# Arthur151/ROMP

Measured on NVIDIA H100. Metric: frames/sec 512x512 ROMP-HRNet32 (whole hot path), higher is better.
Workload: dtype bf16

## Files before the change

romp_b200/csrc/conv_bottleneck_tc.cu:

```cuda
#include "conv_tc.cuh"
#include "tc_device.cuh"

namespace b200romp {

namespace {

constexpr int kBnThreads = 384;
constexpr int kRowB = 128;
constexpr int kHaloW = 10, kHaloH = 18;
constexpr int kChunks = 4;
constexpr int kRing = 2;
constexpr int kW1Bytes = kChunks * 64 * kRowB;
constexpr int kW2Bytes = 9 * 64 * kRowB;
constexpr int kW3Bytes = 256 * kRowB;
constexpr int kStagePayload = kHaloH * kHaloW * kRowB;
constexpr int kStageBytes = 192 * kRowB;
constexpr int kMidBytes = 192 * kRowB;
constexpr int kT2Bytes = 128 * kRowB;
constexpr int kSmemBytes = kW1Bytes + kW2Bytes + kW3Bytes + kRing * kStageBytes + kMidBytes + kT2Bytes + 1024  +
                           1024 ;
static_assert(kSmemBytes <= 227 * 1024, "fused bottleneck does not fit shared memory");

__device__ __forceinline__ void consumers_bar_sync() { asm volatile("bar.sync 1, 256;" ::: "memory"); }

__device__ __forceinline__ void st_shared_b32(uint32_t addr, uint32_t v) {
  asm volatile("st.shared.b32 [%0], %1;" ::"r"(addr), "r"(v) : "memory");
}
template <typename T>
__device__ __forceinline__ T opaque(T v) {
  uint64_t u = (uint64_t)v;
  asm volatile("mov.b64 %0, %0;" : "+l"(u));
  return (T)u;
}
__device__ __forceinline__ uint32_t pack_bf16x2(float a, float b) {
  const __nv_bfloat162 v = __floats2bfloat162_rn(a, b);
  return *reinterpret_cast<const uint32_t*>(&v);
}

}

template <bool STORE_MIDS>
__global__ void __launch_bounds__(kBnThreads, 1)
conv_bottleneck_tc_kernel(const __grid_constant__ CUtensorMap tmap, const ConvParams p, const uint8_t* __restrict__ w1pack,
                          const uint8_t* __restrict__ w2pack, const uint8_t* __restrict__ w3pack, const float* __restrict__ bias1,
                          const float* __restrict__ bias2, BottleneckMids mids, int tiles_x, int tiles_y, int num_tiles) {
  extern __shared__ uint8_t smem_raw[];
  uint8_t* smem = reinterpret_cast<uint8_t*>((reinterpret_cast<uintptr_t>(smem_raw) + 1023) & ~(uintptr_t)1023);
  uint8_t* sW1 = smem;
  uint8_t* sW2 = sW1 + kW1Bytes;
  uint8_t* sW3 = sW2 + kW2Bytes;
  uint8_t* sA = sW3 + kW3Bytes;
  uint8_t* sMid = sA + kRing * kStageBytes;
  uint8_t* sT2 = sMid + kMidBytes;
  uint64_t* full = reinterpret_cast<uint64_t*>(sT2 + kT2Bytes);
  uint64_t* empty = full + kRing;
  uint64_t* w_full = empty + kRing;

  const int warp = threadIdx.x >> 5;
  if (threadIdx.x == 0) {
    for (int i = 0; i < kRing; ++i) {
      mbar_init(&full[i], 1);
      mbar_init(&empty[i], 8);
    }
    mbar_init(w_full, 1);
    fence_barrier_init();
  }
  __syncthreads();
  pdl_trigger();
  const int per_frame = tiles_x * tiles_y;

  if (warp == 0) {
    if (elect_one()) {
      mbar_arrive_expect_tx(w_full, kW1Bytes + kW2Bytes + kW3Bytes);
      bulk_copy_g2s(sW1, w1pack, kW1Bytes, w_full);
      for (int t = 0; t < 9; ++t) bulk_copy_g2s(sW2 + t * 64 * kRowB, w2pack + (size_t)t * 64 * kRowB, 64 * kRowB, w_full);
      bulk_copy_g2s(sW3, w3pack, kW3Bytes, w_full);
      pdl_wait();
      const uint64_t pol = l2_policy_stream();
      int stage = 0;
      uint32_t phase = 0;
      for (int tile = blockIdx.x; tile < num_tiles; tile += gridDim.x) {
        const int n = tile / per_frame, rem = tile % per_frame;
        const int y0 = (rem / tiles_x) * 16, x0 = (rem % tiles_x) * 8;
        for (int c = 0; c < kChunks; ++c) {
          mbar_wait(&empty[stage], phase ^ 1);
          mbar_arrive_expect_tx(&full[stage], kStagePayload);
          tma_load_4d(sA + stage * kStageBytes, &tmap, &full[stage], c * 64, x0 - 1, y0 - 1, n, pol);
          if (++stage == kRing) { stage = 0; phase ^= 1; }
        }
      }
    }
  } else if (warp >= 4) {
    const int g = (warp >> 2) - 1, t = threadIdx.x & 127, w = t >> 5, l = t & 31;
    pdl_wait();
    mbar_wait(w_full, 0);
    const int cl = 2 * (l & 3);
    int stage = 0;
    uint32_t phase = 0;
    for (int tile = blockIdx.x; tile < num_tiles; tile += gridDim.x) {
      const uint32_t w1_base = opaque(smem_u32(sW1)), w2_base = opaque(smem_u32(sW2)), w3_base = opaque(smem_u32(sW3)),
                     a_base = opaque(smem_u32(sA)), mid_base = opaque(smem_u32(sMid)), t2_base = opaque(smem_u32(sT2));
      const float* b1p = opaque(bias1);
      const float* b2p = opaque(bias2);
      const float* b3p = opaque(p.bias);
      const int n = tile / per_frame, rem = tile % per_frame;
      const int y0 = (rem / tiles_x) * 16, x0 = (rem % tiles_x) * 8;

      float acc[32], acc_b[16];
#pragma unroll
      for (int j = 0; j < 32; ++j) acc[j] = 0.f;
#pragma unroll
      for (int j = 0; j < 16; ++j) acc_b[j] = 0.f;
      uint32_t scale_d = 0;
      int prev = -1;
#pragma unroll
      for (int c = 0; c < kChunks; ++c) {
        mbar_wait(&full[stage], phase);
        const uint32_t a_st = a_base + (uint32_t)(stage * kStageBytes);
        const uint32_t b_ch = w1_base + (uint32_t)(c * 64 * kRowB);
        wgmma_fence();
#pragma unroll
        for (int k = 0; k < 4; ++k) {
          wgmma_n64(acc, make_smem_desc(a_st + 64 * g * kRowB + k * 32, 8 * kRowB, kSw128),
                    make_smem_desc(b_ch + k * 32, 8 * kRowB, kSw128), scale_d, false);
          wgmma_n32(acc_b, make_smem_desc(a_st + 128 * kRowB + k * 32, 8 * kRowB, kSw128),
                    make_smem_desc(b_ch + 32 * g * kRowB + k * 32, 8 * kRowB, kSw128), scale_d, false);
          scale_d = 1;
        }
        wgmma_commit();
        if (prev >= 0) {
          wgmma_wait<1>();
          if (l == 0) mbar_arrive(&empty[prev]);
        }
        prev = stage;
        if (++stage == kRing) { stage = 0; phase ^= 1; }
      }
      wgmma_wait<0>();
      if (l == 0) mbar_arrive(&empty[prev]);

      consumers_bar_sync();
      auto mid_store = [&](int m, int j, float a, float b) {
        const int my = m / kHaloW, mx = m % kHaloW;
        const bool inside = my < kHaloH && (unsigned)(y0 - 1 + my) < (unsigned)p.Hout && (unsigned)(x0 - 1 + mx) < (unsigned)p.Wout;
        if (!inside) a = b = 0.f;
        const uint32_t v = pack_bf16x2(a, b);
        st_shared_b32(mid_base + m * kRowB + ((j ^ (m & 7)) << 4) + 2 * cl, v);
        if constexpr (STORE_MIDS) {
          if (mids.t1 != nullptr && my >= 1 && my <= 16 && mx >= 1 && mx <= 8) {
            const size_t pix = ((size_t)n * p.Hout + y0 - 1 + my) * p.Wout + x0 - 1 + mx;
            *reinterpret_cast<uint32_t*>(mids.t1 + pix * mids.t1_C + 8 * j + cl) = v;
          }
        }
      };
#pragma unroll
      for (int e = 0; e < 2; ++e) {
        const int m = 64 * g + 16 * w + (l >> 2) + 8 * e;
#pragma unroll
        for (int j = 0; j < 8; ++j) {
          const int c = 8 * j + cl;
          mid_store(m, j, fmaxf(acc[4 * j + 2 * e] + __ldg(b1p + c), 0.f), fmaxf(acc[4 * j + 2 * e + 1] + __ldg(b1p + c + 1), 0.f));
        }
        const int mb = 128 + 16 * w + (l >> 2) + 8 * e;
#pragma unroll
        for (int j = 0; j < 4; ++j) {
          const int c = 32 * g + 8 * j + cl;
          mid_store(mb, 4 * g + j, fmaxf(acc_b[4 * j + 2 * e] + __ldg(b1p + c), 0.f),
                    fmaxf(acc_b[4 * j + 2 * e + 1] + __ldg(b1p + c + 1), 0.f));
        }
      }
      fence_proxy_async();
      consumers_bar_sync();

      float acc2[32];
#pragma unroll
      for (int j = 0; j < 32; ++j) acc2[j] = 0.f;
      scale_d = 0;
      wgmma_fence();
#pragma unroll
      for (int tap = 0; tap < 9; ++tap) {
        const uint32_t a_tap = mid_base + (uint32_t)(((8 * g + tap / 3) * kHaloW + tap % 3) * kRowB);
        const uint32_t b_tap = w2_base + (uint32_t)(tap * 64 * kRowB);
#pragma unroll
        for (int k = 0; k < 4; ++k) {
          wgmma_n64(acc2, make_smem_desc(a_tap + k * 32, kHaloW * kRowB, kSw128), make_smem_desc(b_tap + k * 32, 8 * kRowB, kSw128),
                    scale_d, false);
          scale_d = 1;
        }
      }
      wgmma_commit();
      wgmma_wait<0>();

#pragma unroll
      for (int e = 0; e < 2; ++e) {
        const int m = 64 * g + 16 * w + (l >> 2) + 8 * e;
#pragma unroll
        for (int j = 0; j < 8; ++j) {
          const int c = 8 * j + cl;
          const uint32_t v = pack_bf16x2(fmaxf(acc2[4 * j + 2 * e] + __ldg(b2p + c), 0.f), fmaxf(acc2[4 * j + 2 * e + 1] + __ldg(b2p + c + 1), 0.f));
          st_shared_b32(t2_base + m * kRowB + ((j ^ (m & 7)) << 4) + 2 * cl, v);
          if constexpr (STORE_MIDS) {
            if (mids.t2 != nullptr) {
              const size_t pix = ((size_t)n * p.Hout + y0 + 8 * g + 2 * w + e) * p.Wout + x0 + (l >> 2);
              *reinterpret_cast<uint32_t*>(mids.t2 + pix * mids.t2_C + c) = v;
            }
          }
        }
      }
      fence_proxy_async();
      wg_bar_sync(2 + g);

      const __nv_bfloat16* res = reinterpret_cast<const __nv_bfloat16*>(p.res);
      __nv_bfloat16* out = reinterpret_cast<__nv_bfloat16*>(p.out);
#pragma unroll 1
      for (int h = 0; h < 2; ++h) {
        float acc3[64];
#pragma unroll
        for (int j = 0; j < 64; ++j) acc3[j] = 0.f;
        wgmma_fence();
#pragma unroll
        for (int k = 0; k < 4; ++k)
          wgmma_n128_bf16(acc3, make_smem_desc(t2_base + 64 * g * kRowB + k * 32, 8 * kRowB, kSw128),
                          make_smem_desc(w3_base + h * 128 * kRowB + k * 32, 8 * kRowB, kSw128), k > 0 ? 1u : 0u);
        wgmma_commit();
        uint32_t rv[2][16];
#pragma unroll
        for (int e = 0; e < 2; ++e) {
          const size_t pix = ((size_t)n * p.Hout + y0 + 8 * g + 2 * w + e) * p.Wout + x0 + (l >> 2);
          const uint32_t* r = reinterpret_cast<const uint32_t*>(res + pix * p.res_C + p.res_c_off + 128 * h + cl);
#pragma unroll
          for (int j = 0; j < 16; ++j) rv[e][j] = r[4 * j];
        }
        wgmma_wait<0>();
#pragma unroll
        for (int e = 0; e < 2; ++e) {
          const size_t pix = ((size_t)n * p.Hout + y0 + 8 * g + 2 * w + e) * p.Wout + x0 + (l >> 2);
          __nv_bfloat162* o = reinterpret_cast<__nv_bfloat162*>(out + pix * p.out_C + p.out_c_off + 128 * h + cl);
#pragma unroll
          for (int j = 0; j < 16; ++j) {
            const int c = 128 * h + 8 * j + cl;
            float a = acc3[4 * j + 2 * e] + __ldg(b3p + c), b = acc3[4 * j + 2 * e + 1] + __ldg(b3p + c + 1);
            const float2 r = res_pair(rv[e][j]);
            a += r.x; b += r.y;
            o[4 * j] = __floats2bfloat162_rn(fmaxf(a, 0.f), fmaxf(b, 0.f));
          }
        }
      }
    }
  }
}

bool tc_bottleneck_supported(const ConvParams& p) {
  if (p.in_dtype != B200ROMP_BF16 || p.out_dtype != B200ROMP_BF16 || p.res_dtype != B200ROMP_BF16) return false;
  if (p.cin != 256 || p.cout != 256 || p.up != 1 || p.out_nchw || p.pow_channel >= 0 || p.input_norm || !p.relu) return false;
  if (p.Hin != p.Hout || p.Win != p.Wout || p.Hout % 16 != 0 || p.Wout % 8 != 0) return false;
  if (p.in_C % 8 != 0 || p.in_c_off % 8 != 0 || p.out_C % 8 != 0 || p.out_c_off % 8 != 0) return false;
  if (p.res != p.in || p.res_C != p.in_C || p.res_c_off != p.in_c_off || p.res_broadcast) return false;
  return (reinterpret_cast<uintptr_t>(p.in) & 15) == 0;
}

int tc_bottleneck_prepare(const ConvParams& p, const float* w1_oihw, const float* b1, const float* w2_oihw, const float* b2,
                          const float* w3_oihw, int sm_count, TcConvPlan* plan, std::vector<void*>* allocs) {
  plan->kind = 70;
  plan->eb = 2;
  plan->cin = plan->cout = 256;
  plan->nt = 256;
  plan->grid_x = sm_count;
  plan->grid_y = 1;
  plan->stages = kRing;
  plan->smem_bytes = kSmemBytes;
  int rc = tc_pack_weights(w1_oihw, 256, 64, 1, 64, &plan->d_wpack, allocs, kRowB, 2);
  if (!rc) rc = tc_pack_weights(w2_oihw, 64, 64, 9, 64, &plan->d_wpack2, allocs, kRowB, 2);
  if (!rc) rc = tc_pack_weights(w3_oihw, 64, 256, 1, 256, &plan->d_wpack3, allocs, kRowB, 2);
  if (rc) return rc;
  plan->d_bias1 = static_cast<const float*>(upload(b1, 64 * sizeof(float), allocs));
  plan->d_bias2 = static_cast<const float*>(upload(b2, 64 * sizeof(float), allocs));
  if (!plan->d_bias1 || !plan->d_bias2) return B200ROMP_ECUDA;
  rc = tc_encode_nhwc_input(&plan->tmap_in, p, 2, 64, kHaloW, kHaloH, CU_TENSOR_MAP_SWIZZLE_128B, "conv_bottleneck_tc");
  if (rc) return rc;
  B2R_CUDA_OK(cudaFuncSetAttribute(conv_bottleneck_tc_kernel<false>, cudaFuncAttributeMaxDynamicSharedMemorySize, kSmemBytes));
  B2R_CUDA_OK(cudaFuncSetAttribute(conv_bottleneck_tc_kernel<true>, cudaFuncAttributeMaxDynamicSharedMemorySize, kSmemBytes));
  return B200ROMP_OK;
}

int tc_bottleneck_launch(const TcConvPlan& plan, const ConvParams& p, const BottleneckMids& mids, cudaStream_t stream) {
  const int tiles_x = p.Wout / 8, tiles_y = p.Hout / 16;
  const int num_tiles = tiles_x * tiles_y * p.B;
  const dim3 grid(std::min(plan.grid_x, num_tiles));
  auto kern = mids.t1 != nullptr || mids.t2 != nullptr ? conv_bottleneck_tc_kernel<true> : conv_bottleneck_tc_kernel<false>;
  B2R_CUDA_OK(tc_launch(kern, grid, kBnThreads, plan.smem_bytes, stream, plan.tmap_in, p, reinterpret_cast<const uint8_t*>(plan.d_wpack),
                        reinterpret_cast<const uint8_t*>(plan.d_wpack2), reinterpret_cast<const uint8_t*>(plan.d_wpack3),
                        plan.d_bias1, plan.d_bias2, mids, tiles_x, tiles_y, num_tiles));
  return B200ROMP_OK;
}

}
```

Baseline: 3602.

## Overlap next-tile conv1 with conv3 epilogue, rebalance registers, vectorize residual I/O

The fused bottleneck kernel now starts the first two conv1 chunks of the next tile right after conv2, so the TMA ring and the tensor cores stay busy during the conv2/conv3 epilogues. Producer warps give up registers via setmaxnreg and consumers gain them, to fit the larger live state. The residual loads and output stores move from 32-bit scattered accesses to 128-bit vectors, using a quad shuffle transpose, and an alignment check on the output pointer is added. The cost is more register pressure, extra shuffles, and a more complex ring-phase ordering across tiles.

```diff
diff --git a/romp_b200/csrc/conv_bottleneck_tc.cu b/romp_b200/csrc/conv_bottleneck_tc.cu
--- a/romp_b200/csrc/conv_bottleneck_tc.cu
+++ b/romp_b200/csrc/conv_bottleneck_tc.cu
@@ -31,6 +31,19 @@
   uint64_t u = (uint64_t)v;
   asm volatile("mov.b64 %0, %0;" : "+l"(u));
   return (T)u;
+}
+constexpr int kProducerRegs = 40, kConsumerRegs = 232;
+template <int R>
+__device__ __forceinline__ void setmaxnreg_dec() { asm volatile("setmaxnreg.dec.sync.aligned.u32 %0;" ::"n"(R)); }
+template <int R>
+__device__ __forceinline__ void setmaxnreg_inc() { asm volatile("setmaxnreg.inc.sync.aligned.u32 %0;" ::"n"(R)); }
+__device__ __forceinline__ void quad_transpose(uint32_t (&m)[4], int q) {
+  const bool b1 = q & 2, b0 = q & 1;
+  uint32_t s0 = __shfl_xor_sync(0xffffffffu, b1 ? m[0] : m[2], 2), s1 = __shfl_xor_sync(0xffffffffu, b1 ? m[1] : m[3], 2);
+  if (b1) { m[0] = s0; m[1] = s1; } else { m[2] = s0; m[3] = s1; }
+  s0 = __shfl_xor_sync(0xffffffffu, b0 ? m[0] : m[1], 1);
+  s1 = __shfl_xor_sync(0xffffffffu, b0 ? m[2] : m[3], 1);
+  if (b0) { m[0] = s0; m[2] = s1; } else { m[1] = s0; m[3] = s1; }
 }
 __device__ __forceinline__ uint32_t pack_bf16x2(float a, float b) {
   const __nv_bfloat162 v = __floats2bfloat162_rn(a, b);
@@ -69,8 +82,9 @@
   pdl_trigger();
   const int per_frame = tiles_x * tiles_y;
 
-  if (warp == 0) {
-    if (elect_one()) {
+  if (warp < 4) {
+    setmaxnreg_dec<kProducerRegs>();
+    if (warp == 0 && elect_one()) {
       mbar_arrive_expect_tx(w_full, kW1Bytes + kW2Bytes + kW3Bytes);
       bulk_copy_g2s(sW1, w1pack, kW1Bytes, w_full);
       for (int t = 0; t < 9; ++t) bulk_copy_g2s(sW2 + t * 64 * kRowB, w2pack + (size_t)t * 64 * kRowB, 64 * kRowB, w_full);
@@ -90,53 +104,60 @@
         }
       }
     }
-  } else if (warp >= 4) {
+  } else {
+    setmaxnreg_inc<kConsumerRegs>();
     const int g = (warp >> 2) - 1, t = threadIdx.x & 127, w = t >> 5, l = t & 31;
     pdl_wait();
     mbar_wait(w_full, 0);
     const int cl = 2 * (l & 3);
     int stage = 0;
     uint32_t phase = 0;
+    float acc[32], acc_b[16];
+    auto conv1_chunks = [&](int c0, int c1) {
+      const uint32_t w1_base = opaque(smem_u32(sW1)), a_base = opaque(smem_u32(sA));
+      if (c0 == 0) {
+#pragma unroll
+        for (int j = 0; j < 32; ++j) acc[j] = 0.f;
+#pragma unroll
+        for (int j = 0; j < 16; ++j) acc_b[j] = 0.f;
+      }
+      int prev = -1;
+#pragma unroll
+      for (int c = c0; c < c1; ++c) {
+        mbar_wait(&full[stage], phase);
+        const uint32_t a_st = a_base + (uint32_t)(stage * kStageBytes);
+        const uint32_t b_ch = w1_base + (uint32_t)(c * 64 * kRowB);
+        wgmma_fence();
+#pragma unroll
+        for (int k = 0; k < 4; ++k) {
+          const uint32_t scale_d = c > 0 || k > 0 ? 1u : 0u;
+          wgmma_n64(acc, make_smem_desc(a_st + 64 * g * kRowB + k * 32, 8 * kRowB, kSw128),
+                    make_smem_desc(b_ch + k * 32, 8 * kRowB, kSw128), scale_d, false);
+          wgmma_n32(acc_b, make_smem_desc(a_st + 128 * kRowB + k * 32, 8 * kRowB, kSw128),
+                    make_smem_desc(b_ch + 32 * g * kRowB + k * 32, 8 * kRowB, kSw128), scale_d, false);
+        }
+        wgmma_commit();
+        if (prev >= 0) {
+          wgmma_wait<1>();
+          if (l == 0) mbar_arrive(&empty[prev]);
+        }
+        prev = stage;
+        if (++stage == kRing) { stage = 0; phase ^= 1; }
+      }
+      wgmma_wait<0>();
+      if (l == 0) mbar_arrive(&empty[prev]);
+    };
+    if (blockIdx.x < num_tiles) conv1_chunks(0, kRing);
     for (int tile = blockIdx.x; tile < num_tiles; tile += gridDim.x) {
-      const uint32_t w1_base = opaque(smem_u32(sW1)), w2_base = opaque(smem_u32(sW2)), w3_base = opaque(smem_u32(sW3)),
-                     a_base = opaque(smem_u32(sA)), mid_base = opaque(smem_u32(sMid)), t2_base = opaque(smem_u32(sT2));
+      const uint32_t w2_base = opaque(smem_u32(sW2)), w3_base = opaque(smem_u32(sW3)), mid_base = opaque(smem_u32(sMid)),
+                     t2_base = opaque(smem_u32(sT2));
       const float* b1p = opaque(bias1);
       const float* b2p = opaque(bias2);
       const float* b3p = opaque(p.bias);
       const int n = tile / per_frame, rem = tile % per_frame;
       const int y0 = (rem / tiles_x) * 16, x0 = (rem % tiles_x) * 8;
 
-      float acc[32], acc_b[16];
-#pragma unroll
-      for (int j = 0; j < 32; ++j) acc[j] = 0.f;
-#pragma unroll
-      for (int j = 0; j < 16; ++j) acc_b[j] = 0.f;
-      uint32_t scale_d = 0;
-      int prev = -1;
-#pragma unroll
-      for (int c = 0; c < kChunks; ++c) {
-        mbar_wait(&full[stage], phase);
-        const uint32_t a_st = a_base + (uint32_t)(stage * kStageBytes);
-        const uint32_t b_ch = w1_base + (uint32_t)(c * 64 * kRowB);
-        wgmma_fence();
-#pragma unroll
-        for (int k = 0; k < 4; ++k) {
-          wgmma_n64(acc, make_smem_desc(a_st + 64 * g * kRowB + k * 32, 8 * kRowB, kSw128),
-                    make_smem_desc(b_ch + k * 32, 8 * kRowB, kSw128), scale_d, false);
-          wgmma_n32(acc_b, make_smem_desc(a_st + 128 * kRowB + k * 32, 8 * kRowB, kSw128),
-                    make_smem_desc(b_ch + 32 * g * kRowB + k * 32, 8 * kRowB, kSw128), scale_d, false);
-          scale_d = 1;
-        }
-        wgmma_commit();
-        if (prev >= 0) {
-          wgmma_wait<1>();
-          if (l == 0) mbar_arrive(&empty[prev]);
-        }
-        prev = stage;
-        if (++stage == kRing) { stage = 0; phase ^= 1; }
-      }
-      wgmma_wait<0>();
-      if (l == 0) mbar_arrive(&empty[prev]);
+      conv1_chunks(kRing, kChunks);
 
       consumers_bar_sync();
       auto mid_store = [&](int m, int j, float a, float b) {
@@ -174,7 +195,7 @@
       float acc2[32];
 #pragma unroll
       for (int j = 0; j < 32; ++j) acc2[j] = 0.f;
-      scale_d = 0;
+      uint32_t scale_d = 0;
       wgmma_fence();
 #pragma unroll
       for (int tap = 0; tap < 9; ++tap) {
@@ -189,6 +210,7 @@
       }
       wgmma_commit();
       wgmma_wait<0>();
+      if (tile + (int)gridDim.x < num_tiles) conv1_chunks(0, kRing);
 
 #pragma unroll
       for (int e = 0; e < 2; ++e) {
@@ -222,26 +244,34 @@
           wgmma_n128_bf16(acc3, make_smem_desc(t2_base + 64 * g * kRowB + k * 32, 8 * kRowB, kSw128),
                           make_smem_desc(w3_base + h * 128 * kRowB + k * 32, 8 * kRowB, kSw128), k > 0 ? 1u : 0u);
         wgmma_commit();
-        uint32_t rv[2][16];
+        const int q = l & 3;
+        uint4 rv[2][4];
 #pragma unroll
         for (int e = 0; e < 2; ++e) {
           const size_t pix = ((size_t)n * p.Hout + y0 + 8 * g + 2 * w + e) * p.Wout + x0 + (l >> 2);
-          const uint32_t* r = reinterpret_cast<const uint32_t*>(res + pix * p.res_C + p.res_c_off + 128 * h + cl);
-#pragma unroll
-          for (int j = 0; j < 16; ++j) rv[e][j] = r[4 * j];
+          const uint4* r = reinterpret_cast<const uint4*>(res + pix * p.res_C + p.res_c_off + 128 * h + 8 * q);
+#pragma unroll
+          for (int jj = 0; jj < 4; ++jj) rv[e][jj] = r[4 * jj];
         }
         wgmma_wait<0>();
 #pragma unroll
         for (int e = 0; e < 2; ++e) {
           const size_t pix = ((size_t)n * p.Hout + y0 + 8 * g + 2 * w + e) * p.Wout + x0 + (l >> 2);
-          __nv_bfloat162* o = reinterpret_cast<__nv_bfloat162*>(out + pix * p.out_C + p.out_c_off + 128 * h + cl);
-#pragma unroll
-          for (int j = 0; j < 16; ++j) {
-            const int c = 128 * h + 8 * j + cl;
-            float a = acc3[4 * j + 2 * e] + __ldg(b3p + c), b = acc3[4 * j + 2 * e + 1] + __ldg(b3p + c + 1);
-            const float2 r = res_pair(rv[e][j]);
-            a += r.x; b += r.y;
-            o[4 * j] = __floats2bfloat162_rn(fmaxf(a, 0.f), fmaxf(b, 0.f));
+          uint4* o = reinterpret_cast<uint4*>(out + pix * p.out_C + p.out_c_off + 128 * h + 8 * q);
+#pragma unroll
+          for (int jj = 0; jj < 4; ++jj) {
+            uint32_t rw[4] = {rv[e][jj].x, rv[e][jj].y, rv[e][jj].z, rv[e][jj].w}, ow[4];
+            quad_transpose(rw, q);
+#pragma unroll
+            for (int i = 0; i < 4; ++i) {
+              const int j = 4 * jj + i, c = 128 * h + 8 * j + cl;
+              float a = acc3[4 * j + 2 * e] + __ldg(b3p + c), b = acc3[4 * j + 2 * e + 1] + __ldg(b3p + c + 1);
+              const float2 r = res_pair(rw[i]);
+              a += r.x; b += r.y;
+              ow[i] = pack_bf16x2(fmaxf(a, 0.f), fmaxf(b, 0.f));
+            }
+            quad_transpose(ow, q);
+            o[4 * jj] = make_uint4(ow[0], ow[1], ow[2], ow[3]);
           }
         }
       }
@@ -255,7 +285,7 @@
   if (p.Hin != p.Hout || p.Win != p.Wout || p.Hout % 16 != 0 || p.Wout % 8 != 0) return false;
   if (p.in_C % 8 != 0 || p.in_c_off % 8 != 0 || p.out_C % 8 != 0 || p.out_c_off % 8 != 0) return false;
   if (p.res != p.in || p.res_C != p.in_C || p.res_c_off != p.in_c_off || p.res_broadcast) return false;
-  return (reinterpret_cast<uintptr_t>(p.in) & 15) == 0;
+  return (reinterpret_cast<uintptr_t>(p.in) & 15) == 0 && (reinterpret_cast<uintptr_t>(p.out) & 15) == 0;
 }
 
 int tc_bottleneck_prepare(const ConvParams& p, const float* w1_oihw, const float* b1, const float* w2_oihw, const float* b2,
```

Measured after the change: 3670, median of 6. +1.9%, better.
